# r4dl/StopThePop-Rasterization

Hardware: AMD Instinct MI355X
Metric: fwd+bwd frames/sec at 1920×1080, 1M Gaussians; PSNR vs reference (higher is better)
Workload: dtype f32

## Files before the change

### stopthepop-rasterization_amd/csrc/stp_buffers.hip

```cpp
#include "stp_internal.h"
#include "stp_layout_cache.h"

#include <cstring>
#include <mutex>
#include <string>

namespace stp {

GeometryState carve_geometry(char* base, size_t P, bool with_inv, size_t* total, NamedOffset* names, int* n_names)
{
    Carver c(base);
    GeometryState g{};
    size_t off;
    int n = 0;
    auto note = [&](const char* nm, size_t o, size_t cnt) { if (names) names[n] = {nm, o, cnt}; n++; };
    g.status = c.take<uint32_t>(64, &off);
    g.depths = c.take<float>(P, &off); note("depths", off, P);
    g.clamped = c.take<uint8_t>(3 * P, &off); note("clamped", off, 3 * P);
    g.internal_radii = c.take<int32_t>(P, &off); note("radii", off, P);
    g.rects2D = c.take<float2>(P, &off); note("rects2D", off, 2 * P);
    g.means2D = c.take<float2>(P, &off); note("means2D", off, 2 * P);
    g.cov3D = c.take<float>(6 * P, &off); note("cov3D", off, 6 * P);
    if (with_inv) { g.cov3D_inv = c.take<float4>(3 * P, &off); note("cov3D_inv", off, 12 * P); }
    if (with_inv) { g.gpack = c.take<float4>(4 * P, &off); note("gpack", off, 16 * P); }
    g.conic_opacity = c.take<float4>(P, &off); note("conic_opacity", off, 4 * P);
    g.rgb = c.take<float>(3 * P, &off); note("rgb", off, 3 * P);
    g.tiles_touched = c.take<uint32_t>(P, &off); note("tiles_touched", off, P);
    g.point_offsets = c.take<uint32_t>(P, &off); note("point_offsets", off, P);
    g.block_sums = c.take<uint32_t>((P + 255) / 256, &off);
    g.block_prefix = c.take<uint32_t>((P + 255) / 256, &off);
    g.scan_temp_bytes = scan_temp_bytes(P);
    g.scan_temp = c.take<char>(g.scan_temp_bytes);
    g.invz = c.take<float>(P, &off); note("invz", off, P);
    if (total) *total = c.total();
    if (n_names) *n_names = n;
    return g;
}

ImageState carve_image(char* base, int W, int H, int ty0, int ty1, int log_depth, size_t* total, NamedOffset* names, int* n_names)
{
    Carver c(base);
    ImageState s{};
    size_t off;
    int n = 0;
    auto note = [&](const char* nm, size_t o, size_t cnt) { if (names) names[n] = {nm, o, cnt}; n++; };
    const int gx = (W + TILE - 1) / TILE;
    const int py0 = ty0 * TILE < H ? ty0 * TILE : H, py1 = ty1 * TILE < H ? ty1 * TILE : H;
    const size_t N = (size_t)W * (size_t)(py1 > py0 ? py1 - py0 : 0), T = (size_t)gx * (size_t)(ty1 > ty0 ? ty1 - ty0 : 0);
    s.header = c.take<uint32_t>(64, &off); note("header", off, 4);
    s.final_T = c.take<float>(N, &off); note("final_T", off, N);
    s.n_contrib = c.take<uint32_t>(N, &off); note("n_contrib", off, N);
    s.ranges = c.take<uint2>(T, &off); note("ranges", off, 2 * T);
    s.dbg_minmax = c.take<uint32_t>(2, &off); note("dbg_minmax", off, 2);
    s.tile_counts = c.take<uint32_t>(T, &off); note("tile_counts", off, T);
    s.tile_cursor = c.take<uint32_t>(T, &off); note("tile_cursor", off, T);
    s.bin_total = c.take<uint32_t>(2, &off); note("bin_total", off, 2);
    s.tile_flags = c.take<uint32_t>(T, &off); note("tile_flags", off, T);
    const size_t recs_per_tile = 4 * (size_t)blend_log_rows(log_depth) * 64;
    s.log_depth = log_depth;
    if (log_depth > 0) {
        const size_t recs = T * recs_per_tile;
        s.blend_log = c.take<uint32_t>(recs / 2, &off); note("blend_log", off, recs);
    }
    if (total) *total = c.total();
    if (n_names) *n_names = n;
    if (base) {
        const size_t pix0 = (size_t)W * (size_t)py0, tile0 = (size_t)gx * (size_t)ty0;
        s.final_T -= pix0; s.n_contrib -= pix0;
        s.ranges -= tile0; s.tile_counts -= tile0; s.tile_cursor -= tile0; s.tile_flags -= tile0;
        if (s.blend_log) s.blend_log -= tile0 * (recs_per_tile / 2);
    }
    return s;
}

BinningState carve_binning(char* base, size_t R, size_t* total, NamedOffset* names, int* n_names)
{
    Carver c(base);
    BinningState b{};
    size_t off;
    int n = 0;
    auto note = [&](const char* nm, size_t o, size_t cnt) { if (names) names[n] = {nm, o, cnt}; n++; };
    b.header = c.take<uint32_t>(64, &off); note("header", off, 4);
    b.point_list = c.take<uint32_t>(R, &off); note("point_list", off, R);
    b.point_list_unsorted = c.take<uint32_t>(R, &off); note("point_list_unsorted", off, R);
    b.keys = c.take<uint64_t>(R, &off); note("keys", off, R);
    b.keys_unsorted = c.take<uint64_t>(R, &off); note("keys_unsorted", off, R);
// ... 168 lines not shown
```

### stopthepop-rasterization_amd/csrc/stp_internal.h

```cpp
#pragma once

#include <hip/hip_runtime.h>
#include <cstdint>
#include <cstddef>
#include <cstdlib>
#include <string>

#include "../../include/stp_raster.h"
#include "stp_switches.h"

namespace stp {

constexpr int TILE = 16;
constexpr size_t ALIGN = 256;
static_assert(ALIGN == 256, "Switches::carve_skew (stp_switches.h) is masked to a multiple of 256");
constexpr int MAX_DEVICES = 32;

enum SortMode { MODE_GLOBAL = 0, MODE_FULL = 1, MODE_KBUFFER = 2, MODE_HIER = 3 };
enum SortOrder { ORDER_Z = 0, ORDER_DISTANCE = 1, ORDER_PTD_CENTER = 2, ORDER_PTD_MAX = 3 };

inline bool uses_blend_log(const StpSettings& s)
{
    return s.record_blend_log != 0 && s.debug_visualization == 0 && (s.sort_mode == MODE_HIER || s.sort_mode == MODE_KBUFFER);
}

inline int subtile_mask_kind(const StpSettings& s)
{
    if (s.sort_mode == MODE_HIER && s.hierarchical_4x4_culling) return 1;
    return s.sort_mode == MODE_KBUFFER ? 2 : 0;
}

inline bool requires_depth_along_ray(const StpSettings& s)
{
    return s.sort_mode != MODE_GLOBAL || s.sort_order == ORDER_PTD_CENTER || s.sort_order == ORDER_PTD_MAX;
}

struct Carver {
    char* base;
    size_t off = 0;
    explicit Carver(char* b) : base(b) {}
    static size_t skew() { return switches().carve_skew; }
    template <typename T> T* take(size_t count, size_t* off_out = nullptr)
    {
        off = (off + ALIGN - 1) & ~(ALIGN - 1);
        if (off) off += skew();
        if (off_out) *off_out = off;
        T* p = base ? reinterpret_cast<T*>(base + off) : nullptr;
        off += count * sizeof(T);
        return p;
    }
    size_t total() const { return ((off + ALIGN - 1) & ~(ALIGN - 1)) + ALIGN; }
};

struct GeometryState {
    uint32_t* status;
    float* depths;
    uint8_t* clamped;
    int32_t* internal_radii;
    float2* rects2D;
    float2* means2D;
    float* cov3D;
    float4* cov3D_inv;
    float4* gpack;
    float4* conic_opacity;
    float* rgb;
    uint32_t* tiles_touched;
    uint32_t* point_offsets;
    uint32_t* block_sums;
    uint32_t* block_prefix;
    char* scan_temp;
    size_t scan_temp_bytes;
    float* invz;
};

struct ImageState {
    float* final_T;
    uint32_t* n_contrib;
    uint2* ranges;
    uint32_t* dbg_minmax;
    uint32_t* tile_counts;
    uint32_t* tile_cursor;
    uint32_t* bin_total;
    uint32_t* header;
    uint32_t* tile_flags;
    uint32_t* blend_log;
    int log_depth;
};

struct BinningState {
    uint32_t* header;
    uint32_t* point_list;
    uint32_t* point_list_unsorted;
    uint64_t* keys;
    uint64_t* keys_unsorted;
    char* sort_temp;
    size_t sort_temp_bytes;
    float4* entA;
    float4* entB;
    float4* entC;
    float4* entD;
    float4* entF;
};

constexpr uint32_t STP_HEADER_MAGIC_BINNING = 0x42505453u, STP_HEADER_MAGIC_IMAGE = 0x49505453u;
struct NamedOffset { const char* name; size_t offset; size_t count; };

GeometryState carve_geometry(char* base, size_t P, bool with_inv, size_t* total, NamedOffset* names = nullptr, int* n_names = nullptr);
ImageState carve_image(char* base, int W, int H, int ty0, int ty1, int log_depth , size_t* total, NamedOffset* names = nullptr, int* n_names = nullptr);
BinningState carve_binning(char* base, size_t R, size_t* total, NamedOffset* names = nullptr, int* n_names = nullptr);
void clamp_tile_rows(int height, int& y0, int& y1);

int fail(int code, const std::string& msg);
int fail_hip(hipError_t e, const char* what);
#define STP_TRY(expr, what) do { hipError_t _e = (expr); if (_e != hipSuccess) return fail_hip(_e, what); } while (0)
#define STP_DEBUG_SYNC(what)  STP_TRY(debug ? hipStreamSynchronize(st) : hipSuccess, what)

void timer_begin_forward();
void timer_begin_backward();
void timer_mark(int i, hipStream_t st);

void remember_layout(const void* binning, uint32_t count, int64_t R);
void remember_log_depth(const void* image, uint32_t depth, int64_t R);
int layout_of(const char* binning, uint32_t R, uint32_t* cap, hipStream_t st = nullptr, bool have_stream = false);
int log_depth_of(const char* image, int64_t R, uint32_t* depth, hipStream_t st = nullptr, bool have_stream = false);

// ... 135 lines not shown
```

### stopthepop-rasterization_amd/csrc/stp_preprocess.hip

```cpp
#include "stp_internal.h"
#include "stp_device.h"

namespace stp {

namespace {

struct PreArgs {
    int P, D, M, W, H, gx, gy, ty0, ty1;
    float focal_x, focal_y, tan_fovx, tan_fovy, scale_modifier;
    int sort_order, rect_bounding, tight_opacity_bounding, tile_based_culling, proper_ewa_scaling, prefiltered;
    const float* means3D;
    const float* scales;
    const float* rotations;
    const float* opacities;
    const float* shs;
    const float* cov3D_precomp;
    const float* colors_precomp;
    const float* view;
    const float* proj;
    const float* cam;
    int* radii;
    GeometryState g;
    uint32_t* tile_counts;
};

__device__ __forceinline__ void sh_to_rgb(int idx, int deg, float3 mean, float3 cam, const float* __restrict__ sh,
                                          uint8_t* __restrict__ clamped, float* __restrict__ rgb)
{
#pragma clang fp contract(off)
    float dx = mean.x - cam.x, dy = mean.y - cam.y, dz = mean.z - cam.z;
    const float len = sqrtf(dx * dx + dy * dy + dz * dz);
    const float x = dx / len, y = dy / len, z = dz / len;
    float res[3];
#pragma unroll
    for (int ch = 0; ch < 3; ch++) res[ch] = kSH_C0 * sh[ch];
    if (deg > 0) {
#pragma unroll
        for (int ch = 0; ch < 3; ch++)
            res[ch] = res[ch] - (kSH_C1 * y) * sh[3 + ch] + (kSH_C1 * z) * sh[6 + ch] - (kSH_C1 * x) * sh[9 + ch];
        if (deg > 1) {
            const float xx = x * x, yy = y * y, zz = z * z, xy = x * y, yz = y * z, xz = x * z;
#pragma unroll
            for (int ch = 0; ch < 3; ch++)
                res[ch] = res[ch] + (kSH_C2[0] * xy) * sh[12 + ch] + (kSH_C2[1] * yz) * sh[15 + ch] +
                          (kSH_C2[2] * (2.0f * zz - xx - yy)) * sh[18 + ch] + (kSH_C2[3] * xz) * sh[21 + ch] +
                          (kSH_C2[4] * (xx - yy)) * sh[24 + ch];
            if (deg > 2) {
#pragma unroll
                for (int ch = 0; ch < 3; ch++)
                    res[ch] = res[ch] + (kSH_C3[0] * y * (3.0f * xx - yy)) * sh[27 + ch] + (kSH_C3[1] * xy * z) * sh[30 + ch] +
                              (kSH_C3[2] * y * (4.0f * zz - xx - yy)) * sh[33 + ch] +
                              (kSH_C3[3] * z * (2.0f * zz - 3.0f * xx - 3.0f * yy)) * sh[36 + ch] +
                              (kSH_C3[4] * x * (4.0f * zz - xx - yy)) * sh[39 + ch] + (kSH_C3[5] * z * (xx - yy)) * sh[42 + ch] +
                              (kSH_C3[6] * x * (xx - 3.0f * yy)) * sh[45 + ch];
// ... 97 lines not shown
    }
    if (det == 0.0f) return false;
    const float det_inv = 1.f / det;
    const float4 co = make_float4(c2z * det_inv, -c2y * det_inv, c2x * det_inv, opacity * conv_scale);
    if (co.w < ALPHA_THRESHOLD) return false;

    const float thr = log_rounded(co.w / ALPHA_THRESHOLD);
    const float extent = a.tight_opacity_bounding ? (float)fmin(3.33, (double)sqrtf(2.0f * thr)) : 3.33f;
    const float mid = 0.5f * (c2x + c2z);
    const float lambda = mid + sqrtf(fmaxf(0.01f, mid * mid - det));
    const float radius = extent * sqrtf(lambda);
    if (radius <= 0.0f) return false;

    const float* __restrict__ proj = a.proj;
    float ph[4];
#pragma unroll
    for (int j = 0; j < 4; j++) ph[j] = (proj[j] * mean.x + proj[4 + j] * mean.y) + (proj[8 + j] * mean.z + proj[12 + j] * 1.0f);
    const float p_w = 1.0f / (ph[3] + 0.0000001f);
    const float2 mean2D = make_float2(ndc_to_pix(ph[0] * p_w, a.W), ndc_to_pix(ph[1] * p_w, a.H));

    const float ext_x = fminf(a.rect_bounding ? (extent * sqrtf(c2x)) : radius, radius);
    const float ext_y = fminf(a.rect_bounding ? (extent * sqrtf(c2z)) : radius, radius);
    const float2 rect_dims = make_float2(ext_x, ext_y);
    int fx0, fy0, fx1, fy1;
    get_rect(mean2D, rect_dims, a.gx, a.gy, 0, a.gy, fx0, fy0, fx1, fy1);
    if ((fx1 - fx0) * (fy1 - fy0) == 0) return false;
    o.sc = sc_in; o.q = q_in;
    o.mean = mean; o.pv = pv; o.co = co; o.thr = thr; o.radius = radius; o.mean2D = mean2D; o.rect_dims = rect_dims;
#pragma unroll
    for (int k = 0; k < 6; k++) o.c3[k] = c3[k];
    o.fx0 = fx0; o.fy0 = fy0; o.fx1 = fx1; o.fy1 = fy1;
    o.y0 = min(max(fy0, a.ty0), fy1); o.y1 = max(min(fy1, a.ty1), o.y0);
    return true;
}

__global__ void __launch_bounds__(256) preprocess_kernel(const PreArgs a)
{
#pragma clang fp contract(off)
    const int idx = blockIdx.x * blockDim.x + threadIdx.x;
    PreStageA o{};
    bool alive = false;
    if (idx < a.P) {
        a.radii[idx] = 0;
        a.g.tiles_touched[idx] = 0;
        alive = preprocess_stage_a(a, idx, o);
    }

    const int x0 = o.fx0, x1 = o.fx1, y0 = o.y0, y1 = o.y1;
    int tile_count = (x1 - x0) * (y1 - y0);
    int full_count = 1;
    const bool tbc = a.tile_based_culling != 0;
    const int rect_tiles = (o.fx1 - o.fx0) * (o.fy1 - o.fy0);
    const bool coop = alive && tbc && a.tile_counts == nullptr && rect_tiles > COOP_TILES;
    if (alive && tbc && !coop) {
        tile_count = 0;
        full_count = 0;
        for (int y = o.fy0; y < o.fy1; y++)
            for (int x = o.fx0; x < o.fx1; x++) {
                const float2 tmin = make_float2((float)(x * TILE), (float)(y * TILE));
                const float2 tmax = make_float2((float)((x + 1) * TILE - 1), (float)((y + 1) * TILE - 1));
                float2 mp;
                const float f = max_contrib_power_rect(o.co, o.mean2D, tmin, tmax, (float)(TILE - 1), (float)(TILE - 1), mp);
                const int hit = (f <= o.thr) ? 1 : 0;
                full_count += hit;
                const int mine = (y >= y0 && y < y1) ? hit : 0;
                tile_count += mine;
                if (mine && a.tile_counts) atomicAdd(&a.tile_counts[y * a.gx + x], 1u);
            }
    } else if (alive && !tbc && a.tile_counts) {
        for (int y = y0; y < y1; y++)
            for (int x = x0; x < x1; x++) atomicAdd(&a.tile_counts[y * a.gx + x], 1u);
    }
    {
        const int lane = wave_lane();
        unsigned long long todo = __ballot(coop);
        while (todo) {
            const int src = (int)__builtin_ctzll(todo);
            todo &= todo - 1ull;
            const float4 co = make_float4(bcast_f(o.co.x, src), bcast_f(o.co.y, src), bcast_f(o.co.z, src), bcast_f(o.co.w, src));
            const float2 m2 = make_float2(bcast_f(o.mean2D.x, src), bcast_f(o.mean2D.y, src));
            const float thr = bcast_f(o.thr, src);
            const int sx0 = bcast_i(o.fx0, src), sy0 = bcast_i(o.fy0, src), sx1 = bcast_i(o.fx1, src), sy1 = bcast_i(o.fy1, src);
            const int wy0 = bcast_i(o.y0, src), wy1 = bcast_i(o.y1, src);
            const int w = sx1 - sx0, n = w * (sy1 - sy0);
            int full = 0, mine = 0;
            for (int t0 = 0; t0 < n; t0 += 64) {
                const int t = t0 + lane;
                const int ty = t / w, y = sy0 + ty, x = sx0 + (t - ty * w);
                bool hit = false;
                if (t < n) {
                    const float2 tmin = make_float2((float)(x * TILE), (float)(y * TILE));
                    const float2 tmax = make_float2((float)((x + 1) * TILE - 1), (float)((y + 1) * TILE - 1));
                    float2 mp;
                    hit = max_contrib_power_rect(co, m2, tmin, tmax, (float)(TILE - 1), (float)(TILE - 1), mp) <= thr;
                }
                full += (int)__popcll(__ballot(hit));
                mine += (int)__popcll(__ballot(hit && y >= wy0 && y < wy1));
            }
            if (lane == src) { full_count = full; tile_count = mine; }
        }
    }
    uint32_t my_entries = 0u;
    if (alive && full_count != 0) {
        my_entries = (uint32_t)tile_count;

    const float3 mean = o.mean, pv = o.pv;
    const float4 co = o.co;
    const float2 mean2D = o.mean2D, rect_dims = o.rect_dims;
    const float radius = o.radius;
    const float3 cam = make_float3(a.cam[0], a.cam[1], a.cam[2]);

    if (a.g.cov3D_inv != nullptr) {
        const float3 sc = o.sc;
        const float4 q = o.q;
        const Mat3 S = mat_diag(1.f / (a.scale_modifier * fmaxf(1e-3f, sc.x)), 1.f / (a.scale_modifier * fmaxf(1e-3f, sc.y)),
                                1.f / (a.scale_modifier * fmaxf(1e-3f, sc.z)));
        const Mat3 Mm = mat_mul(S, quat_to_mat(q));
        const Mat3 inv = mat_mul(mat_transpose(Mm), Mm);
        const float dx = cam.x - mean.x, dy = cam.y - mean.y, dz = cam.z - mean.z;
        const float ux = (-inv.m[0][0]) * dx + (-inv.m[1][0]) * dy + (-inv.m[2][0]) * dz;
        const float uy = (-inv.m[0][1]) * dx + (-inv.m[1][1]) * dy + (-inv.m[2][1]) * dz;
        const float uz = (-inv.m[0][2]) * dx + (-inv.m[1][2]) * dy + (-inv.m[2][2]) * dz;
        const bool tame = fabsf(inv.m[0][0]) < 1.0e36f && fabsf(inv.m[0][1]) < 1.0e36f && fabsf(inv.m[0][2]) < 1.0e36f &&
                          fabsf(inv.m[1][1]) < 1.0e36f && fabsf(inv.m[1][2]) < 1.0e36f && fabsf(inv.m[2][2]) < 1.0e36f;
        if (!tame) atomicOr(&a.g.status[1], 2u);
        a.g.cov3D_inv[3 * (size_t)idx + 0] = make_float4(inv.m[0][0], inv.m[0][1], inv.m[0][2], 0.0f);
        a.g.cov3D_inv[3 * (size_t)idx + 1] = make_float4(inv.m[1][1], inv.m[1][2], inv.m[2][2], 0.0f);
        a.g.cov3D_inv[3 * (size_t)idx + 2] = make_float4(ux, uy, uz, 0.0f);
    }

    float depth;
    if (a.sort_order == ORDER_Z) depth = pv.z;
    else {
        const float dx = cam.x - mean.x, dy = cam.y - mean.y, dz = cam.z - mean.z;
        depth = sqrtf(dx * dx + dy * dy + dz * dz);
    }
    a.g.depths[idx] = depth;
    a.radii[idx] = (int)ceilf(radius);
    a.g.rects2D[idx] = rect_dims;
    a.g.means2D[idx] = mean2D;
    a.g.conic_opacity[idx] = co;
    a.g.tiles_touched[idx] = (uint32_t)tile_count;
    if (a.g.invz != nullptr) a.g.invz[idx] = 1.0f / pv.z;
    if (a.g.gpack != nullptr) {
        const float4 s0 = a.g.cov3D_inv[3 * (size_t)idx + 0], s1 = a.g.cov3D_inv[3 * (size_t)idx + 1], s2 = a.g.cov3D_inv[3 * (size_t)idx + 2];
        float4* const gp = a.g.gpack + 4 * (size_t)idx;
        gp[0] = make_float4(s0.x, s0.y, s0.z, s1.x);
        gp[1] = make_float4(s1.y, s1.z, s2.x, s2.y);
        gp[2] = make_float4(s2.z, mean2D.x, mean2D.y, 0.0f);
        gp[3] = co;
    }
    }

    if (a.g.block_sums != nullptr) {
        __shared__ uint32_t s_wave_total[4];
        const int lane = wave_lane(), wave = (int)(threadIdx.x >> 6);
        uint32_t v = my_entries;
#pragma unroll
        for (int d = 1; d < 64; d <<= 1) {
            const uint32_t t = (uint32_t)__shfl_up((int)v, d);
            if (lane >= d) v += t;
        }
        if (lane == 63) s_wave_total[wave] = v;
        __syncthreads();
        for (int k = 0; k < wave; k++) v += s_wave_total[k];
        if (idx < a.P) a.g.point_offsets[idx] = v;
        if (threadIdx.x == 255) a.g.block_sums[blockIdx.x] = v;
    }
}

struct ShArgs {
    int P, D, M;
    const float* means3D;
    const float* shs;
    const float* cam;
    const int* radii;
    uint8_t* clamped;
    float* rgb;
    const float* dc;
};

#ifndef STP_SH_BLOCK
#define STP_SH_BLOCK 256
#endif
constexpr int SH_BLOCK = STP_SH_BLOCK;

template <bool SPLIT>
__global__ void __launch_bounds__(SH_BLOCK) sh_color_kernel(const ShArgs a)
{
    extern __shared__ float s_rows[];
    const int tid = (int)threadIdx.x;
    const int base = (int)blockIdx.x * SH_BLOCK;
    const int idx = base + tid;
    const int rows = min(SH_BLOCK, a.P - base);
    const int row_len = 3 * a.M, row_stride = row_len + 1;
    const float* __restrict__ src = a.shs + (size_t)base * (SPLIT ? row_len - 3 : row_len);
    const float* __restrict__ src_dc = SPLIT ? a.dc + (size_t)base * 3 : nullptr;
    const int total = rows * row_len;
    const bool vec = SPLIT ? aligned16(a.dc, row_len > 3 ? a.shs : nullptr) : true;
    const bool fast = row_len == 48 && rows == SH_BLOCK && vec;
    float4 v48[12];
    if constexpr (SPLIT) {
        static_assert(!SPLIT || SH_BLOCK == 256, "split48_* are written for 256 rows");
        if (fast) split48_load(src_dc, src, tid, v48);
// ... 24 lines not shown
        for (int f = tid; f < total; f += SH_BLOCK) {
            const int r = f / row_len, j = f - r * row_len;
            s_rows[r * row_stride + j] = src[f];
        }
    }
    __syncthreads();
    if (my_radius > 0) {
        const float3 cam = make_float3(a.cam[0], a.cam[1], a.cam[2]);
        sh_to_rgb(idx, a.D, mean, cam, s_rows + tid * row_stride, a.clamped, a.rgb);
    }
}

struct DupArgs {
    int P, W, H, gx, gy, ty0, ty1;
    int sort_order, tile_based_culling;
    const float* inv_vp;
    const float* cam;
    const int* radii;
    GeometryState g;
    uint64_t* keys;
    uint32_t* values;
    uint32_t* tile_cursor;
    uint32_t cap;
    int n_gauss_blocks;
    int n_pad_blocks;
    uint32_t* header;
    uint32_t header_cap;
    uint32_t* zero_ptr;
    uint32_t zero_words;
};
constexpr int DUP_PAD_BLOCKS = 128, DUP_ZERO_BLOCKS = 32;

struct DupGaussian { float2 xy; float4 co; float thr; float3 p0, p1, p2; float global_depth; };
__device__ __forceinline__ bool duplicate_tile(const DupArgs& a, const DupGaussian& g, float3 cam, bool tbc, bool eval_max, bool per_tile_depth,
                                               int x, int y, uint64_t& key)
{
#pragma clang fp contract(off)
    const float2 tmin = make_float2((float)(x * TILE), (float)(y * TILE));
    const float2 tmax = make_float2((float)((x + 1) * TILE - 1), (float)((y + 1) * TILE - 1));
    float2 max_pos = make_float2(0, 0);
    float max_fac = 0.0f;
    if (eval_max) max_fac = max_contrib_power_rect(g.co, g.xy, tmin, tmax, (float)(TILE - 1), (float)(TILE - 1), max_pos);
    float depth = g.global_depth;
    if (per_tile_depth) {
        const float2 center = make_float2((tmin.x + tmax.x) * 0.5f, (tmin.y + tmax.y) * 0.5f);
        const float2 target = (a.sort_order == ORDER_PTD_MAX) ? max_pos : center;
        const float3 dir = view_ray(a.inv_vp, cam, target.x, target.y, a.W, a.H);
        depth = fmaxf(0.0f, depth_along_ray(g.p0, g.p1, g.p2, dir) + 8.0f);
    }
    key = make_sort_key((uint32_t)(y * a.gx + x), depth);
    return !tbc || max_fac <= g.thr;
}

__global__ void __launch_bounds__(256) duplicate_kernel(const DupArgs a)
{
#pragma clang fp contract(off)
    if (blockIdx.x == 0 && threadIdx.x == 0 && a.header) { a.header[0] = STP_HEADER_MAGIC_BINNING; a.header[1] = a.header_cap; a.header[2] = ~a.header_cap; a.header[3] = 0u; }
    if ((int)blockIdx.x >= a.n_gauss_blocks + a.n_pad_blocks) {
        uint4* const z = reinterpret_cast<uint4*>(a.zero_ptr);
        for (uint32_t i = ((uint32_t)blockIdx.x - (uint32_t)(a.n_gauss_blocks + a.n_pad_blocks)) * 256u + threadIdx.x; i < a.zero_words / 4u; i += (uint32_t)DUP_ZERO_BLOCKS * 256u)
            z[i] = make_uint4(0u, 0u, 0u, 0u);
        return;
    }
    if ((int)blockIdx.x >= a.n_gauss_blocks) {
        const int nb = a.n_gauss_blocks;
        const uint32_t total = a.g.block_prefix[nb - 1] + a.g.block_sums[nb - 1];
        for (uint64_t i = (uint64_t)total + ((uint32_t)blockIdx.x - (uint32_t)nb) * 256u + threadIdx.x; i < (uint64_t)a.cap; i += (uint64_t)DUP_PAD_BLOCKS * 256u) {
            a.values[i] = 0xFFFFFFFFu;
            a.keys[i] = make_sort_key(INVALID_TILE_ID, FLT_MAX);
        }
        return;
    }
    const int idx = blockIdx.x * blockDim.x + threadIdx.x;
    const bool valid = idx < a.P && a.radii[idx] > 0;
    const bool tbc = a.tile_based_culling != 0;
    const bool per_tile_depth = a.sort_order == ORDER_PTD_CENTER || a.sort_order == ORDER_PTD_MAX;
    const bool eval_max = tbc || a.sort_order == ORDER_PTD_MAX;
    uint32_t off = 0, off_to = 0;
    int x0 = 0, y0 = 0, x1 = 0, y1 = 0;
    DupGaussian g{};
    float3 cam = make_float3(0, 0, 0);
    if (per_tile_depth) cam = make_float3(a.cam[0], a.cam[1], a.cam[2]);
    if (a.g.block_prefix != nullptr) {
        if (idx < a.P) {
            const uint32_t base = a.g.block_prefix[blockIdx.x];
            off = base + (threadIdx.x == 0 ? 0u : a.g.point_offsets[idx - 1]);
            off_to = base + a.g.point_offsets[idx];
        }
        __syncthreads();
        if (idx < a.P) a.g.point_offsets[idx] = off_to;
    } else if (valid) {
        off = (idx == 0) ? 0u : a.g.point_offsets[idx - 1];
        off_to = a.g.point_offsets[idx];
    }
    if (valid) {
        g.xy = a.g.means2D[idx];
        const float2 ext = a.g.rects2D[idx];
        get_rect(g.xy, ext, a.gx, a.gy, a.ty0, a.ty1, x0, y0, x1, y1);
        if (eval_max) {
            g.co = a.g.conic_opacity[idx];
            g.thr = log_rounded(g.co.w / ALPHA_THRESHOLD);
        }
        if (per_tile_depth) {
            g.p0 = f4_xyz(a.g.cov3D_inv[3 * (size_t)idx + 0]);
            g.p1 = f4_xyz(a.g.cov3D_inv[3 * (size_t)idx + 1]);
            g.p2 = f4_xyz(a.g.cov3D_inv[3 * (size_t)idx + 2]);
        }
        g.global_depth = a.g.depths[idx];
    }
    const bool coop = valid && a.tile_cursor == nullptr && (x1 - x0) * (y1 - y0) > COOP_TILES;
    if (valid && !coop) {
        for (int y = y0; y < y1; y++)
            for (int x = x0; x < x1; x++) {
                uint64_t key;
                if (duplicate_tile(a, g, cam, tbc, eval_max, per_tile_depth, x, y, key)) {
                    if (a.tile_cursor) {
                        const uint32_t slot = atomicAdd(&a.tile_cursor[(uint32_t)(key >> 32)], 1u);
                        a.values[slot] = (uint32_t)idx;
                        a.keys[slot] = key;
                    } else if (off < off_to && off < a.cap) {
                        a.values[off] = (uint32_t)idx;
                        a.keys[off] = key;
                    }
                    off++;
                }
            }
        if (!a.tile_cursor)
            for (; off < off_to && off < a.cap; off++) {
                a.values[off] = 0xFFFFFFFFu;
                a.keys[off] = make_sort_key(INVALID_TILE_ID, FLT_MAX);
            }
    }
    const int lane = wave_lane();
    unsigned long long todo = __ballot(coop);
    while (todo) {
        const int src = (int)__builtin_ctzll(todo);
        todo &= todo - 1ull;
        DupGaussian s;
        s.xy = make_float2(bcast_f(g.xy.x, src), bcast_f(g.xy.y, src));
        s.co = make_float4(bcast_f(g.co.x, src), bcast_f(g.co.y, src), bcast_f(g.co.z, src), bcast_f(g.co.w, src));
        s.thr = bcast_f(g.thr, src);
        s.p0 = make_float3(bcast_f(g.p0.x, src), bcast_f(g.p0.y, src), bcast_f(g.p0.z, src));
        s.p1 = make_float3(bcast_f(g.p1.x, src), bcast_f(g.p1.y, src), bcast_f(g.p1.z, src));
        s.p2 = make_float3(bcast_f(g.p2.x, src), bcast_f(g.p2.y, src), bcast_f(g.p2.z, src));
        s.global_depth = bcast_f(g.global_depth, src);
        const int sx0 = bcast_i(x0, src), sy0 = bcast_i(y0, src), sx1 = bcast_i(x1, src), sy1 = bcast_i(y1, src);
// ... 62 lines not shown
        for (int o = 1; o < 64; o <<= 1) { const uint32_t v = __shfl_up(inc, o); if (ln >= o) inc += v; }
        uint32_t run = inc - sum;
        for (int k = 0; k < 4; k++) { h[4 * ln + k] = run; run += c[k]; }
    }
    __syncthreads();
    for (int t = tid; t < T; t += 1024) {
        const uint32_t c = klass(ranges[t].y - ranges[t].x);
        order[atomicAdd(&s_hist[c], 1u)] = (uint32_t)t;
        if (gather_order) { const int x = xcd_of(t); gather_order[8u * atomicAdd(&s_hx[x * 256 + c], 1u) + (uint32_t)x] = (uint32_t)t; }
    }
}

__global__ void __launch_bounds__(256) mark_visible_kernel(int P, const float* __restrict__ means3D, const float* __restrict__ view, uint8_t* __restrict__ present)
{
#pragma clang fp contract(off)
    const int idx = blockIdx.x * blockDim.x + threadIdx.x;
    if (idx >= P) return;
    const float z = view[2] * means3D[3 * (size_t)idx] + view[6] * means3D[3 * (size_t)idx + 1] + view[10] * means3D[3 * (size_t)idx + 2] + view[14] * 1.0f;
    present[idx] = z > 0.2f ? 1 : 0;
}

}

hipError_t launch_preprocess(const FrameParams& f, const GeometryState& g, int* radii, uint32_t* tile_counts, hipStream_t st)
{
    PreArgs a;
    a.P = f.P; a.D = f.D; a.M = f.M; a.W = f.W; a.H = f.H; a.gx = f.gx; a.gy = f.gy; a.ty0 = f.ty0; a.ty1 = f.ty1;
    a.focal_x = f.focal_x; a.focal_y = f.focal_y; a.tan_fovx = f.tan_fovx; a.tan_fovy = f.tan_fovy; a.scale_modifier = f.scale_modifier;
    a.sort_order = f.s.sort_order; a.rect_bounding = f.s.rect_bounding; a.tight_opacity_bounding = f.s.tight_opacity_bounding;
    a.tile_based_culling = f.s.tile_based_culling; a.proper_ewa_scaling = f.s.proper_ewa_scaling; a.prefiltered = f.prefiltered;
    a.means3D = f.means3D; a.scales = f.scales; a.rotations = f.rotations; a.opacities = f.opacities; a.shs = f.shs;
    a.cov3D_precomp = f.cov3D_precomp; a.colors_precomp = f.colors_precomp; a.view = f.viewmatrix; a.proj = f.projmatrix; a.cam = f.cam_pos;
    a.radii = radii; a.g = g; a.tile_counts = tile_counts;
    if (f.out_invdepth == nullptr) a.g.invz = nullptr;
    hipLaunchKernelGGL(preprocess_kernel, dim3((f.P + 255) / 256), dim3(256), 0, st, a);
    return hipGetLastError();
}

hipError_t launch_duplicate(const FrameParams& f, const GeometryState& g, const int* radii, const BinningState& b, uint32_t* tile_cursor, uint32_t cap, uint32_t header_cap,
                            uint32_t* zero_ptr, size_t zero_words, hipStream_t st)
{
    DupArgs a;
    a.P = f.P; a.W = f.W; a.H = f.H; a.gx = f.gx; a.gy = f.gy; a.ty0 = f.ty0; a.ty1 = f.ty1;
    a.sort_order = f.s.sort_order; a.tile_based_culling = f.s.tile_based_culling;
    a.inv_vp = f.inv_viewprojmatrix; a.cam = f.cam_pos; a.radii = radii; a.g = g;
    a.tile_cursor = tile_cursor;
    a.keys = tile_cursor ? b.keys : b.keys_unsorted; a.values = tile_cursor ? b.point_list : b.point_list_unsorted;
    const bool capped = cap != 0xFFFFFFFFu && g.block_prefix != nullptr && tile_cursor == nullptr;
    a.cap = capped ? cap : 0xFFFFFFFFu;
    a.n_gauss_blocks = (f.P + 255) / 256;
    a.n_pad_blocks = capped ? DUP_PAD_BLOCKS : 0;
    a.zero_ptr = zero_ptr; a.zero_words = (uint32_t)zero_words;
    a.header = b.header; a.header_cap = header_cap;
    hipLaunchKernelGGL(duplicate_kernel, dim3(a.n_gauss_blocks + a.n_pad_blocks + (zero_words ? DUP_ZERO_BLOCKS : 0)), dim3(256), 0, st, a);
    return hipGetLastError();
}

hipError_t launch_sh_color(const FrameParams& f, const GeometryState& g, const int* radii, hipStream_t st)
{
    const bool split = f.sh_dc != nullptr;
    if (f.colors_precomp != nullptr || (f.shs == nullptr && !split) || f.M <= 0) return hipSuccess;
    ShArgs a;
    a.P = f.P; a.D = f.D; a.M = f.M; a.means3D = f.means3D; a.shs = f.shs; a.cam = f.cam_pos; a.radii = radii; a.clamped = g.clamped; a.rgb = g.rgb;
    a.dc = f.sh_dc;
    const void* kernel = split ? reinterpret_cast<const void*>(sh_color_kernel<true>) : reinterpret_cast<const void*>(sh_color_kernel<false>);
    const size_t lds = (size_t)SH_BLOCK * (3 * a.M + 1) * sizeof(float);
    if (lds > 64 * 1024) {
        hipError_t e = hipFuncSetAttribute(kernel, hipFuncAttributeMaxDynamicSharedMemorySize, (int)lds);
        if (e != hipSuccess) return e;
    }
    if (split) hipLaunchKernelGGL(sh_color_kernel<true>, dim3((f.P + SH_BLOCK - 1) / SH_BLOCK), dim3(SH_BLOCK), lds, st, a);
    else hipLaunchKernelGGL(sh_color_kernel<false>, dim3((f.P + SH_BLOCK - 1) / SH_BLOCK), dim3(SH_BLOCK), lds, st, a);
    return hipGetLastError();
}

__global__ void mailbox_kernel(const uint32_t* __restrict__ last_offset, const uint32_t* __restrict__ status, volatile uint32_t* mailbox, uint32_t ticket,
                               uint32_t* log_need)
{
    mailbox[0] = *last_offset;
    mailbox[1] = *status;
    mailbox[3] = log_need ? atomicExch(log_need, 0u) : 0u;
    __threadfence_system();
    mailbox[2] = ticket;
    __threadfence_system();
}

__global__ void __launch_bounds__(1024) block_prefix_mailbox_kernel(const uint32_t* __restrict__ block_sums, uint32_t* __restrict__ block_prefix, int n_blocks,
                                                                     const uint32_t* __restrict__ status, volatile uint32_t* mailbox, uint32_t ticket,
                                                                     uint32_t* log_need)
{
    __shared__ uint32_t s_wave_total[16];
    const int tid = (int)threadIdx.x, lane = tid & 63, wave = tid >> 6;
    const int per = (n_blocks + 1023) / 1024, i0 = min(tid * per, n_blocks), i1 = min(i0 + per, n_blocks);
    uint32_t mine = 0u;
    for (int i = i0; i < i1; i++) mine += block_sums[i];
    uint32_t v = mine;
#pragma unroll
    for (int d = 1; d < 64; d <<= 1) {
        const uint32_t t = (uint32_t)__shfl_up((int)v, d);
        if (lane >= d) v += t;
    }
    if (lane == 63) s_wave_total[wave] = v;
    __syncthreads();
    for (int k = 0; k < wave; k++) v += s_wave_total[k];
    uint32_t run = v - mine;
    for (int i = i0; i < i1; i++) { block_prefix[i] = run; run += block_sums[i]; }
    if (tid == 1023) {
// ... 104 lines not shown
```

### stopthepop-rasterization_amd/csrc/stp_switches.h

```cpp
#pragma once
#include <cstddef>
#include <cstdlib>
#include <cstring>

namespace stp {

struct Switches {
    bool tile_local_sort;
    bool atomic_bin;
    bool fused_gather;
    bool two_level_scan;
    bool colour_late;
    bool speculative_binning;
    bool mailbox_spin;
    bool side_stream;
    int fixed_log_depth;
    size_t carve_skew;
    bool tile_order;
    int gather_order;
    enum TileSort { TILE_SORT_AUTO, TILE_SORT_ROCPRIM, TILE_SORT_OWN } tile_sort;
    enum KBuffer { KBUFFER_RING, KBUFFER_TILE, KBUFFER_WAVE } kbuffer;
};

inline const Switches& switches()
{
    static const Switches table = [] {
        const auto is = [](const char* name, const char* value) { const char* e = std::getenv(name); return e && std::strcmp(e, value) == 0; };
        const auto starts_with_0 = [](const char* name) { const char* e = std::getenv(name); return e && e[0] == '0'; };
        const auto number = [](const char* name) { const char* e = std::getenv(name); return e ? std::atoi(e) : 0; };
        Switches s{};
        s.tile_local_sort = !is("STP_SORT", "radix");
        s.atomic_bin = is("STP_SORT", "counters");
        s.fused_gather = !starts_with_0("STP_FUSED_GATHER");
        s.two_level_scan = !is("STP_SCAN", "rocprim");
        s.colour_late = !starts_with_0("STP_COLOUR_LATE");
        s.speculative_binning = !is("STP_BINNING", "exact");
        s.mailbox_spin = !is("STP_MAILBOX", "event");
        s.side_stream = !is("STP_SIDE_STREAM", "0");
        s.fixed_log_depth = number("STP_LOG_DEPTH");
        const char* skew = std::getenv("STP_CARVE_SKEW");
        s.carve_skew = skew ? ((size_t)std::strtoull(skew, nullptr, 0) & ~(size_t)255) : (size_t)0;
        s.tile_order = !starts_with_0("STP_TILE_ORDER");
        s.gather_order = number("STP_GATHER_ORDER");
        s.tile_sort = is("STP_TILE_SORT", "rocprim") ? Switches::TILE_SORT_ROCPRIM : is("STP_TILE_SORT", "own") ? Switches::TILE_SORT_OWN : Switches::TILE_SORT_AUTO;
        s.kbuffer = is("STP_KBUFFER", "tile") ? Switches::KBUFFER_TILE : is("STP_KBUFFER", "wave") ? Switches::KBUFFER_WAVE : Switches::KBUFFER_RING;
        return s;
    }();
    return table;
}

}
```

### stopthepop-rasterization_amd/diff_gaussian_rasterization/_C.py

```python
from __future__ import annotations

import ctypes
import os
from typing import Tuple

import torch

_HERE = os.path.dirname(os.path.abspath(__file__))
_LIB_NAME = "libstp_raster.so"
_lib = None
_host = None


GRAD_RECORD_FLOATS = 16


class StpSettings(ctypes.Structure):
    _fields_ = [(n, ctypes.c_int32) for n in (
        "sort_mode", "sort_order", "queue_tile_4x4", "queue_tile_2x2", "queue_per_pixel",
        "rect_bounding", "tight_opacity_bounding", "tile_based_culling", "hierarchical_4x4_culling",
        "load_balancing", "proper_ewa_scaling", "tile_y0", "tile_y1", "record_blend_log", "debug_visualization")]


_lib_override = None
# ... 361 lines not shown


class StpDensifyRule(ctypes.Structure):
    _fields_ = [(name, ctypes.c_float) for name in ("grad_threshold", "split_size", "min_opacity", "max_screen_size", "max_world_size", "split_shrink")] + \
               [("raw", ctypes.c_int32), ("prune_big", ctypes.c_int32)]


class StpDensifyTensor(ctypes.Structure):
    _fields_ = [(name, ctypes.c_void_p) for name in ("param", "exp_avg", "exp_avg_sq", "param_out", "exp_avg_out", "exp_avg_sq_out")] + \
               [("row", ctypes.c_int32), ("role", ctypes.c_int32)]


DENSIFY_ROLES = {"plain": 0, "xyz": 1, "scaling": 2, "rotation": 3}


def densify_stats(xyz_gradient_accum, denom, max_radii2D, grad2d, radii) -> int:
    _require("stp_densify_stats")
    return int((_host or _native()).densify_stats(xyz_gradient_accum, denom, max_radii2D, grad2d, radii))


def densify_plan(xyz_gradient_accum, denom, scaling, opacity, max_radii2D, rule, raw, prune_big):
    _require("stp_densify_plan")
    return (_host or _native()).densify_plan(xyz_gradient_accum, denom, scaling, opacity, max_radii2D, [float(x) for x in rule], bool(raw), bool(prune_big))


def densify_scan(plan):
    _require("stp_densify_scan")
    offsets, nK, nC, nS = (_host or _native()).densify_scan(plan)
    return offsets, (int(nK), int(nC), int(nS))


def densify_apply(plan, offsets, counts, tensors, roles, exp_avgs, exp_avg_sqs, noise, split_shrink, raw):
    _require("stp_densify_apply")
    out = (_host or _native()).densify_apply(plan, offsets, [int(c) for c in counts], list(tensors), [int(r) for r in roles], list(exp_avgs),
                                             list(exp_avg_sqs), noise, float(split_shrink), bool(raw))
    return list(out[0]), list(out[1]), list(out[2])


def photometric_forward(image, target, want_maps):
    for name in ("stp_photometric_workspace_floats", "stp_photometric_forward", "stp_photometric_backward"):
        _require(name)
    out2, maps = (_host or _native()).photometric_forward(image, target, bool(want_maps))
    return out2, (maps if want_maps else None)


def photometric_backward(image, target, maps, grad_out2):
    _require("stp_photometric_backward")
    return (_host or _native()).photometric_backward(image, target, maps, grad_out2)


_GEOM_TYPES = {"depths": torch.float32, "clamped": torch.uint8, "radii": torch.int32, "rects2D": torch.float32,
               "means2D": torch.float32, "cov3D": torch.float32, "cov3D_inv": torch.float32,
               "conic_opacity": torch.float32, "rgb": torch.float32, "tiles_touched": torch.int32,
               "point_offsets": torch.int32, "invz": torch.float32}
_BIN_TYPES = {"point_list": torch.int32, "point_list_unsorted": torch.int32, "keys": torch.int64, "keys_unsorted": torch.int64}
_IMG_TYPES = {"final_T": torch.float32, "n_contrib": torch.int32, "ranges": torch.int32, "tile_flags": torch.int32,
              "blend_log": torch.int16}


def timing_text(device=None) -> str:
    buf = ctypes.create_string_buffer(512)
    with _on_device(device):
        _load().stp_timing_text(buf, 512)
    return buf.value.decode()


def _view(buf: torch.Tensor, off: int, count: int, dtype) -> torch.Tensor:
    nbytes = count * torch.empty((), dtype=dtype).element_size()
    return buf[off:off + nbytes].view(dtype)


def geometry_array(geomBuffer, P, settings_dict, name):
    s = settings_from_dict(settings_dict)
    off, cnt = ctypes.c_size_t(), ctypes.c_size_t()
    if _load().stp_geometry_layout(int(P), ctypes.byref(s), name.encode(), ctypes.byref(off), ctypes.byref(cnt)) != 0:
        raise KeyError(name)
    return _view(geomBuffer, off.value, cnt.value, _GEOM_TYPES[name])


def binning_array(binningBuffer, R, name):
    off, cnt = ctypes.c_size_t(), ctypes.c_size_t()
    L = _load()
    if binningBuffer.is_cuda:
        _native().forget_unless_same_storage(binningBuffer)
    lay = int(L.stp_binning_layout_count(ctypes.c_void_p(binningBuffer.data_ptr()), int(R))) if int(R) > 0 else 0
    if lay < 0:
        _raise_last(lay)
    if L.stp_binning_layout(lay, name.encode(), ctypes.byref(off), ctypes.byref(cnt)) != 0:
        raise KeyError(name)
    n = cnt.value // lay * int(R) if lay > 0 else cnt.value
    return _view(binningBuffer, off.value, n, _BIN_TYPES[name])


def image_array(imgBuffer, W, H, name, tile_rows=None):
    off, cnt = ctypes.c_size_t(), ctypes.c_size_t()
    L = _load()
    L.stp_image_layout_depth.argtypes = [ctypes.c_int] * 5 + [ctypes.c_char_p, ctypes.POINTER(ctypes.c_size_t), ctypes.POINTER(ctypes.c_size_t)]
    y0, y1 = (0, 0) if tile_rows is None else (int(tile_rows[0]), int(tile_rows[1]))
    depth = blend_log_depth(imgBuffer) if name == "blend_log" else 0
    if L.stp_image_layout_depth(int(W), int(H), y0, y1, depth, name.encode(), ctypes.byref(off), ctypes.byref(cnt)) != 0:
        raise KeyError(name)
    return _view(imgBuffer, off.value, cnt.value, _IMG_TYPES[name])


def blend_log_depth(imgBuffer) -> int:
    L = _load()
    L.stp_blend_log_depth.argtypes = [ctypes.c_void_p]
# ... 59 lines not shown
```

Measured before the change: 456.9.

## Parallelize Gaussian duplication per output entry using preprocess tile masks

Preprocess now records a 64-bit mask of which tiles in each Gaussian's rect pass tile-based culling, and stores depth in the spare gpack slot. A new templated duplicate kernel path stages each workgroup's Gaussians in shared memory and assigns threads to output key/value entries. Each thread finds its owner Gaussian by binary search over the local offsets and its tile by the k-th set bit of the mask. This removes per-Gaussian load imbalance and the repeated culling evaluation during duplication, at the cost of extra shared memory, a per-Gaussian mask buffer and search overhead per entry.

```diff
diff --git a/stopthepop-rasterization_amd/csrc/stp_buffers.hip b/stopthepop-rasterization_amd/csrc/stp_buffers.hip
--- a/stopthepop-rasterization_amd/csrc/stp_buffers.hip
+++ b/stopthepop-rasterization_amd/csrc/stp_buffers.hip
@@ -32,6 +32,7 @@
     g.scan_temp_bytes = scan_temp_bytes(P);
     g.scan_temp = c.take<char>(g.scan_temp_bytes);
     g.invz = c.take<float>(P, &off); note("invz", off, P);
+    g.tile_mask = c.take<uint64_t>(P, &off); note("tile_mask", off, P);
     if (total) *total = c.total();
     if (n_names) *n_names = n;
     return g;
diff --git a/stopthepop-rasterization_amd/csrc/stp_dup_index.h b/stopthepop-rasterization_amd/csrc/stp_dup_index.h
--- /dev/null
+++ b/stopthepop-rasterization_amd/csrc/stp_dup_index.h
@@ -0,0 +1,55 @@
+#pragma once
+#include <cstdint>
+
+#if defined(__HIPCC__)
+#define STP_HD __host__ __device__ __forceinline__
+#else
+#define STP_HD inline
+#endif
+
+namespace stp {
+
+STP_HD int dup_owner_of(const uint32_t* incl, int n, uint32_t e)
+{
+    int j = 0;
+    for (int step = 128; step >= 1; step >>= 1) {
+        const int probe = j + step - 1;
+        if (probe < n && incl[probe] <= e) j += step;
+    }
+    return j;
+}
+
+STP_HD int dup_kth_set_bit(uint64_t m, int k)
+{
+    uint32_t w = (uint32_t)m;
+    int pos = 0;
+    int c = __builtin_popcount(w);
+    if (k >= c) { k -= c; pos = 32; w = (uint32_t)(m >> 32); }
+    c = __builtin_popcount(w & 0xFFFFu);
+    if (k >= c) { k -= c; pos += 16; w >>= 16; }
+    c = __builtin_popcount(w & 0xFFu);
+    if (k >= c) { k -= c; pos += 8; w >>= 8; }
+    c = __builtin_popcount(w & 0xFu);
+    if (k >= c) { k -= c; pos += 4; w >>= 4; }
+    c = __builtin_popcount(w & 0x3u);
+    if (k >= c) { k -= c; pos += 2; w >>= 2; }
+    if (k >= (int)(w & 1u)) pos += 1;
+    return pos;
+}
+
+STP_HD int dup_row_of(int p, int w)
+{
+    int q = (int)((float)p / (float)w);
+    if (q * w > p) q--;
+    if ((q + 1) * w <= p) q++;
+    return q;
+}
+
+STP_HD uint64_t dup_mask_window(uint64_t m, int lo, int n)
+{
+    if (n <= 0 || lo >= 64) return 0ull;
+    m >>= lo;
+    return n >= 64 ? m : (m & ((1ull << n) - 1ull));
+}
+
+}
diff --git a/stopthepop-rasterization_amd/csrc/stp_internal.h b/stopthepop-rasterization_amd/csrc/stp_internal.h
--- a/stopthepop-rasterization_amd/csrc/stp_internal.h
+++ b/stopthepop-rasterization_amd/csrc/stp_internal.h
@@ -71,6 +71,7 @@
     char* scan_temp;
     size_t scan_temp_bytes;
     float* invz;
+    uint64_t* tile_mask;
 };
 
 struct ImageState {
diff --git a/stopthepop-rasterization_amd/csrc/stp_preprocess.hip b/stopthepop-rasterization_amd/csrc/stp_preprocess.hip
--- a/stopthepop-rasterization_amd/csrc/stp_preprocess.hip
+++ b/stopthepop-rasterization_amd/csrc/stp_preprocess.hip
@@ -1,5 +1,6 @@
 #include "stp_internal.h"
 #include "stp_device.h"
+#include "stp_dup_index.h"
 
 namespace stp {
 
@@ -203,17 +204,21 @@
     const bool tbc = a.tile_based_culling != 0;
     const int rect_tiles = (o.fx1 - o.fx0) * (o.fy1 - o.fy0);
     const bool coop = alive && tbc && a.tile_counts == nullptr && rect_tiles > COOP_TILES;
+    uint32_t mask_lo = 0u, mask_hi = 0u;
     if (alive && tbc && !coop) {
         tile_count = 0;
         full_count = 0;
+        int t = 0;
         for (int y = o.fy0; y < o.fy1; y++)
-            for (int x = o.fx0; x < o.fx1; x++) {
+            for (int x = o.fx0; x < o.fx1; x++, t++) {
                 const float2 tmin = make_float2((float)(x * TILE), (float)(y * TILE));
                 const float2 tmax = make_float2((float)((x + 1) * TILE - 1), (float)((y + 1) * TILE - 1));
                 float2 mp;
                 const float f = max_contrib_power_rect(o.co, o.mean2D, tmin, tmax, (float)(TILE - 1), (float)(TILE - 1), mp);
                 const int hit = (f <= o.thr) ? 1 : 0;
                 full_count += hit;
+                if (t < 32) mask_lo |= (uint32_t)hit << t;
+                else if (t < 64) mask_hi |= (uint32_t)hit << (t - 32);
                 const int mine = (y >= y0 && y < y1) ? hit : 0;
                 tile_count += mine;
                 if (mine && a.tile_counts) atomicAdd(&a.tile_counts[y * a.gx + x], 1u);
@@ -298,9 +303,10 @@
         float4* const gp = a.g.gpack + 4 * (size_t)idx;
         gp[0] = make_float4(s0.x, s0.y, s0.z, s1.x);
         gp[1] = make_float4(s1.y, s1.z, s2.x, s2.y);
-        gp[2] = make_float4(s2.z, mean2D.x, mean2D.y, 0.0f);
+        gp[2] = make_float4(s2.z, mean2D.x, mean2D.y, depth);
         gp[3] = co;
     }
+    if (tbc && a.g.tile_mask != nullptr) a.g.tile_mask[idx] = ((uint64_t)mask_hi << 32) | (uint64_t)mask_lo;
     }
 
     if (a.g.block_sums != nullptr) {
@@ -431,6 +437,7 @@
     return !tbc || max_fac <= g.thr;
 }
 
+template <bool ENTRY>
 __global__ void __launch_bounds__(256) duplicate_kernel(const DupArgs a)
 {
 #pragma clang fp contract(off)
@@ -451,7 +458,6 @@
         return;
     }
     const int idx = blockIdx.x * blockDim.x + threadIdx.x;
-    const bool valid = idx < a.P && a.radii[idx] > 0;
     const bool tbc = a.tile_based_culling != 0;
     const bool per_tile_depth = a.sort_order == ORDER_PTD_CENTER || a.sort_order == ORDER_PTD_MAX;
     const bool eval_max = tbc || a.sort_order == ORDER_PTD_MAX;
@@ -460,17 +466,83 @@
     DupGaussian g{};
     float3 cam = make_float3(0, 0, 0);
     if (per_tile_depth) cam = make_float3(a.cam[0], a.cam[1], a.cam[2]);
-    if (a.g.block_prefix != nullptr) {
-        if (idx < a.P) {
-            const uint32_t base = a.g.block_prefix[blockIdx.x];
-            off = base + (threadIdx.x == 0 ? 0u : a.g.point_offsets[idx - 1]);
-            off_to = base + a.g.point_offsets[idx];
-        }
+    bool valid;
+    if constexpr (ENTRY) {
+        __shared__ uint32_t s_off[256];
+        __shared__ float4 s_g[4][256];
+        __shared__ int4 s_rc[256];
+        __shared__ uint64_t s_mask[256];
+        const int tid = (int)threadIdx.x, first = (int)blockIdx.x * 256, n_local = min(256, a.P - first);
+        const int ic = min(idx, a.P - 1);
+        const bool need_co = a.sort_order == ORDER_PTD_MAX;
+        const uint32_t po = a.g.point_offsets[ic];
+        const uint32_t wg_base = a.g.block_prefix != nullptr ? a.g.block_prefix[blockIdx.x] : (first == 0 ? 0u : a.g.point_offsets[first - 1]);
+        float4 r0 = make_float4(0, 0, 0, 0), r1 = r0, r2 = r0, r3 = r0;
+        if (a.g.gpack != nullptr && per_tile_depth) {
+            const float4* __restrict__ gp = a.g.gpack + 4 * (size_t)ic;
+            r0 = gp[0]; r1 = gp[1]; r2 = gp[2];
+            if (need_co) r3 = gp[3];
+        } else {
+            const float2 m = a.g.means2D[ic];
+            r2 = make_float4(0.0f, m.x, m.y, a.g.depths[ic]);
+            if (need_co) r3 = a.g.conic_opacity[ic];
+        }
+        const float2 ext = a.g.rects2D[ic];
+        const uint64_t mask = tbc ? a.g.tile_mask[ic] : 0ull;
+        const uint32_t incl = a.g.block_prefix != nullptr ? po : po - wg_base;
+        s_off[tid] = incl;
         __syncthreads();
-        if (idx < a.P) a.g.point_offsets[idx] = off_to;
-    } else if (valid) {
-        off = (idx == 0) ? 0u : a.g.point_offsets[idx - 1];
-        off_to = a.g.point_offsets[idx];
+        const uint32_t excl = tid == 0 ? 0u : s_off[tid - 1];
+        if (a.g.block_prefix != nullptr && idx < a.P) a.g.point_offsets[idx] = wg_base + incl;
+        const bool has = idx < a.P && incl > excl;
+        int fx0, fy0, fx1, fy1;
+        get_rect(make_float2(r2.y, r2.z), ext, a.gx, a.gy, 0, a.gy, fx0, fy0, fx1, fy1);
+        const int w = fx1 - fx0, wy0 = max(fy0, a.ty0), wy1 = max(min(fy1, a.ty1), wy0);
+        valid = has && tbc && w * (fy1 - fy0) > COOP_TILES;
+        const bool by_entry = has && !valid;
+        s_g[0][tid] = r0; s_g[1][tid] = r1; s_g[2][tid] = r2; s_g[3][tid] = r3;
+        s_rc[tid] = make_int4(fx0, w, wy0, by_entry ? 1 : 0);
+        s_mask[tid] = (by_entry && tbc) ? dup_mask_window(mask, (wy0 - fy0) * w, (wy1 - wy0) * w) : 0ull;
+        __syncthreads();
+        const uint32_t total = s_off[n_local - 1];
+        for (uint32_t e = (uint32_t)tid; e < total; e += 256u) {
+            const int j = dup_owner_of(s_off, n_local, e);
+            const int4 rc = s_rc[j];
+            if (rc.w == 0) continue;
+            const int k = (int)(e - (j == 0 ? 0u : s_off[j - 1]));
+            const int p = tbc ? dup_kth_set_bit(s_mask[j], k) : k;
+            const int ty = dup_row_of(p, rc.y);
+            DupGaussian s;
+            const float4 q2 = s_g[2][j];
+            s.xy = make_float2(q2.y, q2.z);
+            s.global_depth = q2.w;
+            s.co = make_float4(0, 0, 0, 0); s.thr = 0.0f;
+            s.p0 = s.p1 = s.p2 = make_float3(0, 0, 0);
+            if (need_co) s.co = s_g[3][j];
+            if (per_tile_depth) {
+                const float4 q0 = s_g[0][j], q1 = s_g[1][j];
+                s.p0 = make_float3(q0.x, q0.y, q0.z); s.p1 = make_float3(q0.w, q1.x, q1.y); s.p2 = make_float3(q1.z, q1.w, q2.x);
+            }
+            uint64_t key;
+            (void)duplicate_tile(a, s, cam, false, need_co, per_tile_depth, rc.x + (p - ty * rc.y), rc.z + ty, key);
+            const uint32_t slot = wg_base + e;
+            if (slot < a.cap) { a.values[slot] = (uint32_t)(first + j); a.keys[slot] = key; }
+        }
+        off = wg_base + excl; off_to = wg_base + incl;
+    } else {
+        valid = idx < a.P && a.radii[idx] > 0;
+        if (a.g.block_prefix != nullptr) {
+            if (idx < a.P) {
+                const uint32_t base = a.g.block_prefix[blockIdx.x];
+                off = base + (threadIdx.x == 0 ? 0u : a.g.point_offsets[idx - 1]);
+                off_to = base + a.g.point_offsets[idx];
+            }
+            __syncthreads();
+            if (idx < a.P) a.g.point_offsets[idx] = off_to;
+        } else if (valid) {
+            off = (idx == 0) ? 0u : a.g.point_offsets[idx - 1];
+            off_to = a.g.point_offsets[idx];
+        }
     }
     if (valid) {
         g.xy = a.g.means2D[idx];
@@ -639,7 +711,10 @@
     a.n_pad_blocks = capped ? DUP_PAD_BLOCKS : 0;
     a.zero_ptr = zero_ptr; a.zero_words = (uint32_t)zero_words;
     a.header = b.header; a.header_cap = header_cap;
-    hipLaunchKernelGGL(duplicate_kernel, dim3(a.n_gauss_blocks + a.n_pad_blocks + (zero_words ? DUP_ZERO_BLOCKS : 0)), dim3(256), 0, st, a);
+    const bool by_entry = switches().duplicate_entry && tile_cursor == nullptr && (f.s.tile_based_culling == 0 || g.tile_mask != nullptr);
+    const dim3 grid(a.n_gauss_blocks + a.n_pad_blocks + (zero_words ? DUP_ZERO_BLOCKS : 0));
+    if (by_entry) hipLaunchKernelGGL(duplicate_kernel<true>, grid, dim3(256), 0, st, a);
+    else hipLaunchKernelGGL(duplicate_kernel<false>, grid, dim3(256), 0, st, a);
     return hipGetLastError();
 }
 
diff --git a/stopthepop-rasterization_amd/csrc/stp_switches.h b/stopthepop-rasterization_amd/csrc/stp_switches.h
--- a/stopthepop-rasterization_amd/csrc/stp_switches.h
+++ b/stopthepop-rasterization_amd/csrc/stp_switches.h
@@ -9,6 +9,7 @@
     bool tile_local_sort;
     bool atomic_bin;
     bool fused_gather;
+    bool duplicate_entry;
     bool two_level_scan;
     bool colour_late;
     bool speculative_binning;
@@ -32,6 +33,7 @@
         s.tile_local_sort = !is("STP_SORT", "radix");
         s.atomic_bin = is("STP_SORT", "counters");
         s.fused_gather = !starts_with_0("STP_FUSED_GATHER");
+        s.duplicate_entry = !is("STP_DUPLICATE", "gaussian");
         s.two_level_scan = !is("STP_SCAN", "rocprim");
         s.colour_late = !starts_with_0("STP_COLOUR_LATE");
         s.speculative_binning = !is("STP_BINNING", "exact");
diff --git a/stopthepop-rasterization_amd/diff_gaussian_rasterization/_C.py b/stopthepop-rasterization_amd/diff_gaussian_rasterization/_C.py
--- a/stopthepop-rasterization_amd/diff_gaussian_rasterization/_C.py
+++ b/stopthepop-rasterization_amd/diff_gaussian_rasterization/_C.py
@@ -437,7 +437,7 @@
 _GEOM_TYPES = {"depths": torch.float32, "clamped": torch.uint8, "radii": torch.int32, "rects2D": torch.float32,
                "means2D": torch.float32, "cov3D": torch.float32, "cov3D_inv": torch.float32,
                "conic_opacity": torch.float32, "rgb": torch.float32, "tiles_touched": torch.int32,
-               "point_offsets": torch.int32, "invz": torch.float32}
+               "point_offsets": torch.int32, "invz": torch.float32, "tile_mask": torch.int64}
 _BIN_TYPES = {"point_list": torch.int32, "point_list_unsorted": torch.int32, "keys": torch.int64, "keys_unsorted": torch.int64}
 _IMG_TYPES = {"final_T": torch.float32, "n_contrib": torch.int32, "ranges": torch.int32, "tile_flags": torch.int32,
               "blend_log": torch.int16}
```

Result: no change. 460.5 (median of 4 runs) (+0.8%).
